# nanoporetech/isONclust2

Measured on AMD Instinct MI355X. Metric: reads/s clustered (sahlin mode, k=11 w=15), higher is better.
Workload: dtype u32

## Files before the change

isonclust2_amd/csrc/ioc_align_gpu.hip:

```cpp
#include <hip/hip_runtime.h>

#include <algorithm>
#include <chrono>
#include <cmath>
#include <cstdint>
#include <cstring>
#include <numeric>
#include <string>
#include <type_traits>
#include <vector>

#include "ioc_align_sink.h"
#include "ioc_internal.h"

namespace {

constexpr int ALN_C = 8;
constexpr int ALN_MAXW = 8;
constexpr int ALN_NEG = INT32_MIN / 4;
constexpr uint32_t ALN_LEN_SHIFT = 26;

struct AlnPairDev {
    uint32_t q_off, n;
    uint32_t r_off, m;
// ... 779 lines not shown
            const int2 x = mylrow[e];
            if (x.x > br || (x.x == br && uint32_t(x.y) < bj)) {
                br = x.x;
                bj = uint32_t(x.y);
            }
        }
        for (int o = 32; o > 0; o >>= 1) {
            const int s = __shfl_xor(br, o);
            const uint32_t j = __shfl_xor(bj, o);
            if (s > br || (s == br && j < bj)) {
                br = s;
                bj = j;
            }
        }
        if (lane == 0) {
            int fin = ALN_NEG;
            uint32_t bi = 0, bjj = m;
            for (uint32_t b2 = 0; b2 < nwaves; ++b2) {
                if (min(n, b2 * tpb * TILE) >= n) break;
                const int2 bb = cross ? X.best[uint64_t(pslot - X.first_pair) * nwaves + b2] : int2{s_best[slot * wpp + b2][0], s_best[slot * wpp + b2][1]};
                if (bb.x > fin) {
                    fin = bb.x;
                    bi = uint32_t(bb.y);
                }
            }
            if (br > fin) {
                fin = br;
                bi = n;
                bjj = bj;
            }
            ends[pid] = int4{fin, int(bi), int(bjj), 0};
        }
    }
}

struct WinStat {
    uint32_t wb = 0, pushed = 0, cnt = 0;
    __device__ __forceinline__ void push(uint32_t bit, uint32_t kmask, uint32_t k, int il)
    {
        wb = ((wb << 1) | bit) & kmask;
        ++pushed;
        if (pushed > k && int(__popc(wb)) >= il) ++cnt;
    }
    __device__ __forceinline__ void push_run(unsigned long long bits, uint32_t m, uint32_t kmask, uint32_t k, int il, uint32_t lane)
    {
        const unsigned long long upto = __brevll(bits << (63u - lane));
        const unsigned long long old = lane + 1u < 64u ? (unsigned long long)wb << (lane + 1u) : 0ull;
        const uint32_t win = uint32_t(old | upto) & kmask;
        const bool hit = lane < m && pushed + lane + 1u > k && int(__popc(win)) >= il;
        cnt += uint32_t(__popcll(__ballot(hit)));
        wb = uint32_t(__builtin_amdgcn_readlane(int(win), int(m - 1u)));
        pushed += m;
    }
    __device__ void blanks(uint32_t g, uint32_t kmask, uint32_t k, int il)
    {
        const uint32_t t = g < k ? g : k;
        for (uint32_t x = 0; x < t; ++x) push(0u, kmask, k, il);
        if (g > t) {
            const uint32_t rest = g - t;
            const uint32_t first_counted = pushed >= k ? 0u : k - pushed;
            pushed += rest;
            if (il <= 0 && rest > first_counted) cnt += rest - first_counted;
        }
    }
};

struct AlnOpsDev {
    uint8_t* buf;
    const uint64_t* end;
    uint32_t* len;
};

struct NoOpsDev {};
template <bool EMIT>
struct OpsOut {
    using Dev = NoOpsDev;
    __device__ __forceinline__ void begin(Dev, uint32_t, uint32_t) {}
    __device__ __forceinline__ void run(unsigned long long, uint32_t, uint32_t) {}
    __device__ __forceinline__ void step(uint8_t, uint32_t) {}
    __device__ __forceinline__ void fill(uint8_t, uint32_t, uint32_t) {}
    __device__ __forceinline__ void end(Dev, uint32_t, uint32_t) {}
    __device__ __forceinline__ void none(Dev, uint32_t) {}
};
template <>
struct OpsOut<true> {
    using Dev = AlnOpsDev;
    uint8_t* cur = nullptr;
    uint8_t* lo = nullptr;
    __device__ __forceinline__ void begin(const Dev& od, uint32_t pid, uint32_t room)
    {
        cur = od.buf + od.end[pid];
        lo = cur - room;
    }
    __device__ __forceinline__ void run(unsigned long long bits, uint32_t m, uint32_t lane)
    {
        if (lane < m && cur - 1 - lane >= lo) cur[-1 - int(lane)] = (bits >> lane) & 1ull ? uint8_t('=') : uint8_t('X');
        cur -= m;
    }
    __device__ __forceinline__ void step(uint8_t op, uint32_t lane)
    {
        if (lane == 0 && cur > lo) cur[-1] = op;
        cur -= 1;
    }
    __device__ __forceinline__ void fill(uint8_t op, uint32_t g, uint32_t lane)
    {
        const uint64_t room = uint64_t(cur > lo ? cur - lo : 0);
        for (uint32_t x = lane; x < g && x < room; x += 64) cur[-1 - int64_t(x)] = op;
// ... 685 lines not shown
    std::vector<uint32_t> rw(size_t(np) * V2_RESUME_WORDS);
    IOC_CHK(c, hipMemcpy(rw.data(), t.resume, rw.size() * 4, hipMemcpyDeviceToHost));
    std::vector<uint32_t> ids(n_pairs);
    for (uint32_t x = 0; x < n_pairs; ++x) ids[x] = order[first_pair + x];
    auto rec = [&](uint32_t pid, uint32_t w) { return rw[size_t(pid) * V2_RESUME_WORDS + w]; };
    auto cost = [&](uint32_t pid) { return (double(rec(pid, 8)) + double(rec(pid, 12))) * 256.0; };
    std::sort(ids.begin(), ids.end(), [&](uint32_t a, uint32_t b) { return cost(a) > cost(b); });
    double sum = 0;
    uint32_t parked = 0;
    for (uint32_t pid : ids) {
        sum += cost(pid);
        parked += rec(pid, 6) ? 1u : 0u;
    }
    fprintf(stderr, "[ioc] k_trace2: %u pairs, %u walks went on in the second launch (deadline %u blocks); mean %.3e cycles (s_memtime), slowest first:\n", n_pairs, parked,
            deadline, sum / n_pairs);
    auto line = [&](const char* tag, uint32_t pid) {
        const AlnPairDev& d = dp[pid];
        fprintf(stderr, "[ioc]   %s pair %u: %.3e + %.3e cycles, n %u m %u, blocks %u (%u on the diagonal) + %u (%u by helpers), tiles %u + %u, gap steps %u, windows %u\n", tag, pid,
                double(rec(pid, 8)) * 256.0, double(rec(pid, 12)) * 256.0, d.n, d.m, rec(pid, 9) & 0xFFFFu, rec(pid, 9) >> 16, rec(pid, 13) & 0xFFFFu, rec(pid, 13) >> 16,
                rec(pid, 10), rec(pid, 14), rec(pid, 11), rec(pid, 15));
    };
    {
        double pk_max = -1e9, un_min = 1e9, pk_sum = 0, un_sum = 0;
        uint32_t npk = 0, nun = 0;
        std::vector<double> pks, uns;
        for (uint32_t pid : ids) {
            const AlnPairDev& d = dp[pid];
            const double q = double(he[pid].x) / double(std::max(1u, std::min(d.n, d.m)));
            if (rec(pid, 6)) {
                pk_max = std::max(pk_max, q), pk_sum += q, ++npk;
                pks.push_back(q);
            } else {
                un_min = std::min(un_min, q), un_sum += q, ++nun;
                uns.push_back(q);
            }
        }
        std::sort(pks.begin(), pks.end());
        std::sort(uns.begin(), uns.end());
        auto qt = [](const std::vector<double>& v, double f) { return v.empty() ? 0.0 : v[std::min(v.size() - 1, size_t(f * double(v.size())))]; };
        fprintf(stderr, "[ioc]   forward score / shorter length: parked walks (%u) mean %.3f, 50 %% %.3f, 90 %% %.3f, 99 %% %.3f, max %.3f | others (%u) min %.3f, 1 %% %.3f, 10 %% %.3f, mean %.3f\n", npk,
                npk ? pk_sum / npk : 0.0, qt(pks, 0.5), qt(pks, 0.9), qt(pks, 0.99), pk_max, nun, un_min, qt(uns, 0.01), qt(uns, 0.1), nun ? un_sum / nun : 0.0);
    }
    for (uint32_t x = 0; x < std::min(n_pairs, 10u); ++x) line("", ids[x]);
    for (uint32_t qx : {n_pairs / 4u, n_pairs / 2u, 3u * n_pairs / 4u}) line("rank", ids[qx]);
    std::vector<uint32_t> sw(size_t(np) * V2_SPLIT_WORDS);
    IOC_CHK(c, hipMemcpy(sw.data(), t.split, sw.size() * 4, hipMemcpyDeviceToHost));
    for (uint32_t l = 0; l < 2u; ++l) {
        auto cyc = [&](uint32_t pid) { return double(rec(pid, l ? 12 : 8)) * 256.0; };
        auto spl = [&](uint32_t pid, uint32_t w) { return sw[size_t(pid) * V2_SPLIT_WORDS + l * (V2_SPLIT_WORDS / 2u) + w]; };
        std::vector<uint32_t> in;
        for (uint32_t pid : ids)
            if (rec(pid, l ? 12 : 8)) in.push_back(pid);
        std::sort(in.begin(), in.end(), [&](uint32_t a, uint32_t b) { return cyc(a) > cyc(b); });
        double tot[8] = {};
        for (uint32_t pid : in) {
            tot[0] += cyc(pid);
            for (uint32_t w = 0; w < 3u; ++w) tot[1 + w] += double(spl(pid, w)) * 256.0;
            tot[4] += double(spl(pid, 3) & 0xFFFFu);
            tot[5] += double(spl(pid, 4));
            tot[6] += double(spl(pid, 5));
            tot[7] += double(spl(pid, 6));
        }
        const double nn = double(std::max<size_t>(1, in.size()));
        fprintf(stderr, "[ioc] split of %s: %zu walks; mean %.3e cycles: blocks %.1f %%, tile recomputation %.1f %%, walk loop %.1f %%; %.1f cycles per tile step; "
                        "blocks of <= 64 columns: %.2f per walk, %.1f %% of the block steps recomputed by walkers\n",
                l ? "k_trace2_help" : "k_trace2", in.size(), tot[0] / nn, 100.0 * tot[1] / std::max(1.0, tot[0]), 100.0 * tot[2] / std::max(1.0, tot[0]),
                100.0 * tot[3] / std::max(1.0, tot[0]), tot[2] / std::max(1.0, tot[7]), tot[4] / nn, 100.0 * tot[6] / std::max(1.0, tot[5]));
        for (size_t x = 0; x < std::min<size_t>(in.size(), 10); ++x) {
            const uint32_t pid = in[x];
            const uint32_t nb = l ? rec(pid, 13) & 0xFFFFu : rec(pid, 9) & 0xFFFFu;
            fprintf(stderr, "[ioc]   split pair %u: %.3e cycles: blocks %.3e, tiles %.3e, walk %.3e; blocks %u (<= 64 columns %u, <= 64 rows %u), own block steps %u (%u in thin), tiles %u, tile steps %u\n",
                    pid, cyc(pid), double(spl(pid, 0)) * 256.0, double(spl(pid, 1)) * 256.0, double(spl(pid, 2)) * 256.0, nb, spl(pid, 3) & 0xFFFFu, spl(pid, 3) >> 16,
                    spl(pid, 4), spl(pid, 5), rec(pid, l ? 14 : 10), spl(pid, 6));
        }
    }
    return IOC_OK;
}

int align_v2_run(ioc_ctx* c, const std::vector<AlnPairDev>& dp, const uint32_t* order, uint32_t cnt, const uint32_t* d_order,
                 const AlnParams& P, int32_t* d_score, uint32_t* d_count, bool corridor, bool* fell_back, OpsRun* ops)
{
    *fell_back = false;
    if (cnt == 0) return IOC_OK;
    int r;
    const auto t_plan0 = std::chrono::steady_clock::now();
    V2Opts o{};
    o.n_cu = compute_units(c);
    uint64_t budget = 0;
    if ((r = ck_budget(c, &budget, ops ? ops->host->pile_bytes() : 0)) != IOC_OK) return r;
    o.guard = P16_GUARD;
    if (const char* e = getenv("IOC_ALIGN_V2_GUARD")) o.guard = std::max(1, std::min(P16_GUARD, atoi(e)));
    o.few_limit = 128;
    if (const char* e = getenv("IOC_ALIGN_V2_FEW")) o.few_limit = uint32_t(std::max(0, atoi(e)));
    if (hipOccupancyMaxActiveBlocksPerMultiprocessor(&o.occ, reinterpret_cast<const void*>(k_fwd2), 64 * V2_WAVES, 0) != hipSuccess) o.occ = 0;
    (void)hipGetLastError();
    if (o.occ < 1) o.occ = 3;

    V2Plan pl;
    pl.cnt = cnt;
    pl.np = uint32_t(dp.size());
    pl.ncouples = (cnt + 1u) / 2u;
    plan_couples(pl, dp, order, corridor_model(c, P, corridor), band_target(pl.ncouples, o.few_limit, o.occ, o.n_cu));
    std::vector<uint64_t> cops;
    if (ops) {
        cops.assign(pl.ncouples, 0);
        for (uint32_t x = 0; x < cnt; ++x) cops[x / 2u] += uint64_t(dp[order[x]].n) + dp[order[x]].m;
    }
    slice_couples(pl, budget, cops);
    std::vector<uint64_t> slice_ops(pl.slices.size(), 0);
    if (ops) {
        ops->end.assign(dp.size(), 0);
        uint64_t most = 0;
        for (size_t si = 0; si < pl.slices.size(); ++si) {
            const uint32_t x0 = 2u * pl.slices[si].first, x1 = std::min(cnt, 2u * (pl.slices[si].first + pl.slices[si].second));
            for (uint32_t x = x0; x < x1; ++x) ops->end[order[x]] = slice_ops[si] += uint64_t(dp[order[x]].n) + dp[order[x]].m;
            most = std::max(most, slice_ops[si]);
        }
        if ((r = ops_reserve(c, *ops, most, dp)) != IOC_OK) return r;
    }
    const auto t_res0 = std::chrono::steady_clock::now();
    IOC_TRY(ioc_reserve(c, c->a_ck, size_t(pl.arena_words) * 4));
    c->tm.align_arena_bytes = int64_t(pl.arena_words) * 4;
    c->tm.align_slices = int32_t(pl.slices.size());
    c->tm.align_version = 2;
    if (getenv("IOC_TRACE"))
        fprintf(stderr, "[ioc]   aligner v2: %u couples, checkpoint arena %.1f MB (%zu slice(s)) reserved in %.3f ms; corridor: %llu of %llu tiles skipped\n", pl.ncouples,
// ... 668 lines not shown
```

isonclust2_amd/csrc/ioc_align_v2.inc:

```

constexpr int CK2 = 512;
constexpr int V2_WAVES = 4;
constexpr int V2_BLK_C = 8;
constexpr int V2_MAX_BANDS = 40;
static_assert(CK2 % TILE == 0 && CK2 == 64 * V2_BLK_C, "block geometry");

struct V2Couple {
    uint32_t pid[2];
    uint32_t nbands, nstrips;
    uint32_t tpb;
    uint32_t flag0;
    uint32_t mpad;
    uint32_t nq;
    uint64_t rdat;
    uint64_t rbase;
    uint64_t cdat;
    uint64_t cbase;
    uint64_t prof;
    uint32_t lrow0[2];
    uint32_t best0[2];
    uint16_t bstart[V2_MAX_BANDS + 1];
    uint16_t plo[V2_MAX_BANDS], phi[V2_MAX_BANDS];
    uint32_t corridor;
    uint16_t probe_band, probe_strip;
// ... 600 lines not shown
        };
        {
            uint32_t s = 0;
            for (; s + 1u < nsteps; s += 2) {
                step(s, std::true_type{});
                step(s + 1u, std::false_type{});
            }
            for (; s < nsteps; ++s) step(s, std::true_type{});
        }
#pragma unroll
        for (int h = 0; h < 2; ++h) {
            if (lastc[h] >= 0) bandbest[par(VP_BEST0 + h) + band] = int2{bc[h], int(bc_i[h])};
            if ((ovf >> h) & 1u) {
                const uint32_t pidh = par(VP_PID0 + h);
                if (pidh != 0xFFFFFFFFu) atomicOr(&ovf_out[pidh], 1u);
            }
        }
        if (lane == 0) {
            unsigned long long cells = 0;
#pragma unroll
            for (int h = 0; h < 2; ++h)
                if (vh[h]) cells += (unsigned long long)(par(VP_RHI0 + h) - r_lo) * (unsigned long long)min(strip_cols, par(VP_M0 + h) - p * strip_cols);
            atomicAdd(cells_done, cells);
        }
        const uint32_t my_flag = uint32_t(__builtin_amdgcn_readfirstlane(int(par(VP_FLAG))));
        asm volatile("s_waitcnt vmcnt(0)" ::: "memory");
        __builtin_amdgcn_fence(__ATOMIC_RELEASE, "agent");
        asm volatile("s_waitcnt vmcnt(0)" ::: "memory");
        __hip_atomic_store(&flags[my_flag], 1u, __ATOMIC_RELAXED, __HIP_MEMORY_SCOPE_AGENT);
        it = v2_dequeue(queue);
    }
}

#define V2_FWD_ARGS                                                                                                                        \
    const AlnPairDev *__restrict__ pairs, const V2Couple *__restrict__ couples, const V2Item *__restrict__ items, uint32_t n_items,        \
        uint32_t *__restrict__ queue, uint32_t *__restrict__ flags, uint32_t *__restrict__ err, const uint8_t *__restrict__ pool, AlnParams P, \
        uint32_t *__restrict__ arena, int2 *__restrict__ lrow, int2 *__restrict__ bandbest, uint32_t *__restrict__ ovf_out, int guard,     \
        const uint4 *__restrict__ prof, unsigned long long *__restrict__ cells_done, uint32_t *__restrict__ prog, uint32_t prog_every
__global__ void __launch_bounds__(64 * V2_WAVES) __attribute__((amdgpu_waves_per_eu(3, 8))) k_fwd2(V2_FWD_ARGS)
{
    v2_fwd_body(pairs, couples, items, n_items, queue, flags, err, pool, P, arena, lrow, bandbest, ovf_out, guard, prof, cells_done, prog, prog_every);
}
__global__ void __launch_bounds__(64 * V2_WAVES) __attribute__((amdgpu_waves_per_eu(2, 2))) k_fwd2_w2(V2_FWD_ARGS)
{
    v2_fwd_body(pairs, couples, items, n_items, queue, flags, err, pool, P, arena, lrow, bandbest, ovf_out, guard, prof, cells_done, prog, prog_every);
}


struct V2PairEnd {
    uint32_t lrow0, best0, nbands, couple;
    int32_t cert;
};
constexpr uint32_t V2_RESUME_WORDS = 16;
constexpr uint32_t V2_SPLIT_WORDS = 16;

__global__ void __launch_bounds__(64)
k_fwd2_probe(const AlnPairDev* __restrict__ pairs, V2Couple* __restrict__ couples, V2PairEnd* __restrict__ pe, const uint32_t* __restrict__ arena, AlnParams P)
{
    V2Couple& cp = couples[blockIdx.x];
    if (!cp.corridor) return;
    const uint32_t lane = threadIdx.x;
    const uint32_t strip_cols = 64u * FW_C;
    const uint32_t R = uint32_t(cp.bstart[cp.probe_band + 1u]) * uint32_t(CK2);
    const uint32_t ckr = R / uint32_t(CK2) - 1u;
    const uint32_t* rh = arena + cp.rdat + uint64_t(2u * ckr) * cp.mpad;
    const int2* rb = reinterpret_cast<const int2*>(arena + cp.rbase) + uint64_t(ckr) * (cp.mpad / 16u);
    bool wrong = false;
    uint32_t nmax = 0, mmax = 0, need = 0, need_raw = 0;
    for (int h = 0; h < 2; ++h) {
        if (cp.pid[h] == 0xFFFFFFFFu) continue;
        const AlnPairDev pr = pairs[cp.pid[h]];
        nmax = max(nmax, pr.n);
        mmax = max(mmax, pr.m);
        const int gd = pr.gap_open - P.gap_extend;
        int mx = INT32_MIN;
        const uint32_t x0 = uint32_t(cp.probe_strip) * strip_cols, x1 = min(pr.m, x0 + strip_cols);
        for (uint32_t x = x0 + lane; x < x1; x += 64) {
            const int2 bb = rb[x / 16u];
            mx = max(mx, v2_half(rh[x], h) + (h ? bb.y : bb.x) + gd - P.gap_extend * int(R + x + 1u));
        }
        for (int o = 32; o > 0; o >>= 1) mx = max(mx, __shfl_xor(mx, o));
        if (pr.n < R || x1 <= x0 || mx < P.match * int(R) / 4) {
            wrong = true;
        } else {
            const float len = float(max(pr.n, pr.m)), rate = float(mx) / float(R);
            const float b = len - 0.97f * rate * float(min(pr.n, pr.m)) / float(P.match) + 512.0f;
            need = max(need, uint32_t(max(b, 0.0f)));
            need_raw = max(need_raw, uint32_t(max(len - rate * float(min(pr.n, pr.m)) / float(P.match), 0.0f)));
        }
    }
    const uint32_t len_max = max(nmax, mmax);
    const uint32_t B0 = cp.b0;
    if (!wrong && need_raw > B0 && need > B0) {
        if (float(need) > 0.4f * float(len_max)) {
            wrong = true;
        } else if (lane == 0) {
            long long beff = 0x7FFFFFFFFFFFll;
            uint32_t skipped = 0;
            for (uint32_t b = 0; b < cp.nbands; ++b) {
                const uint32_t r0 = uint32_t(cp.bstart[b]) * uint32_t(CK2), r1 = min(nmax, uint32_t(cp.bstart[b + 1u]) * uint32_t(CK2));
                const uint32_t c_lo = r0 > need ? r0 - need : 0u;
                const unsigned long long c_hi = min((unsigned long long)mmax, (unsigned long long)r1 + need);
                const uint32_t lo = c_lo / strip_cols, hi = uint32_t((max(c_hi, 1ull) - 1ull) / strip_cols);
                cp.plo[b] = uint16_t(min(lo, uint32_t(cp.plo[b])));
                cp.phi[b] = uint16_t(max(hi, uint32_t(cp.phi[b])));
                skipped += uint32_t(cp.plo[b]) + (cp.nstrips - 1u - uint32_t(cp.phi[b]));
                if (cp.plo[b] > 0) beff = min(beff, (long long)r0 - (long long)cp.plo[b] * strip_cols);
// ... 88 lines not shown
__device__ __forceinline__ int2 v2_ld(const int2* p)
{
    const int x = __hip_atomic_load(&p->x, __ATOMIC_RELAXED, __HIP_MEMORY_SCOPE_AGENT);
    const int y = __hip_atomic_load(&p->y, __ATOMIC_RELAXED, __HIP_MEMORY_SCOPE_AGENT);
    return int2{x, y};
}

constexpr uint32_t V2_NROLE = 5, V2_NHELP = 2 * V2_NROLE, V2_HBUF = 2, V2_HWAVES = 1 + V2_NHELP;
enum V2Help : uint32_t { VH_SEQ = 0, VH_RB, VH_CB, VH_I, VH_J, VH_QUIT, VH_WORK = 8 , VH_SLOT = VH_WORK + 3 * V2_NHELP ,
                         VH_COUNT = VH_SLOT + 3 * V2_NHELP * V2_HBUF };

template <bool HELP, bool EMIT>
__device__ __forceinline__ void trace2_body(const AlnPairDev* __restrict__ pairs, const uint32_t* __restrict__ order, const uint8_t* __restrict__ pool,
                                            const AlnParams& P, const uint32_t* __restrict__ arena, const V2Couple* __restrict__ couples, const V2PairCk* __restrict__ pck,
                                            const int4* __restrict__ ends, V2Scratch* __restrict__ scratch, V2Scratch* __restrict__ hscratch,
                                            uint32_t* __restrict__ resume, uint32_t* __restrict__ park, uint32_t* __restrict__ split,
                                            int32_t* __restrict__ out_score, uint32_t* __restrict__ out_count, const uint32_t count, const uint32_t max_blocks,
                                            const unsigned long long max_cycles, const uint32_t pslot, const uint32_t wv, const uint32_t want,
                                            const typename OpsOut<EMIT>::Dev od)
{
    constexpr int NW = HELP ? int(V2_HWAVES) : TR_WAVES, NDIRS = HELP ? 1 : TR_WAVES;
    constexpr uint32_t B_LEFT = uint32_t(CK2) * 8u, B_Q = uint32_t(CK2) * 4u, B_PROF = 5u * 64u * uint32_t(V2_BLK_C / 4) * 4u;
    constexpr uint32_t D_BYTES = uint32_t(TILE) * uint32_t(TR_C) / 4u * 64u * 2u;
    constexpr uint32_t U_BYTES = (B_LEFT + B_Q + B_PROF) > D_BYTES + uint32_t(TILE) ? (B_LEFT + B_Q + B_PROF) : D_BYTES + uint32_t(TILE);
    __shared__ __attribute__((aligned(16))) uint8_t s_union_all[NW][U_BYTES];
    __shared__ __attribute__((aligned(16))) uint8_t s_tile_all[NDIRS][uint32_t(TILE) * 12u];
    __shared__ uint32_t s_help[VH_COUNT];
    if (pslot >= count) return;
    uint16_t(*dirs)[64] = reinterpret_cast<uint16_t(*)[64]>(&s_union_all[wv][0]);
    int2* const b_left = reinterpret_cast<int2*>(&s_union_all[wv][0]);
    uint32_t* const b_q = reinterpret_cast<uint32_t*>(&s_union_all[wv][B_LEFT]);
    uint32_t* const b_prof = reinterpret_cast<uint32_t*>(&s_union_all[wv][B_LEFT + B_Q]);
    struct TRec {
        int hq, e;
        uint32_t q;
    };
    static_assert(sizeof(TRec) == 12, "a row's record");
    TRec* const s_rec = reinterpret_cast<TRec*>(&s_tile_all[HELP ? 0u : wv][0]);
    uint8_t* const s_rb = &s_union_all[wv][D_BYTES];
    const uint32_t pid = order[pslot];
    const AlnPairDev pr = pairs[pid];
    const V2PairCk ck = pck[pid];
    const int hf = int(ck.half);
    const bool corridor = __builtin_amdgcn_readfirstlane(int(couples[ck.couple].corridor)) != 0;
    uint32_t* const rs = resume + size_t(pid) * V2_RESUME_WORDS;
    {
        const uint32_t fl = uint32_t(__builtin_amdgcn_readfirstlane(int(rs[6])));
        if (HELP ? fl != want : fl == 2u) return;
    }
    V2Scratch* scp = &scratch[pslot];
    const unsigned long long t_begin = __builtin_amdgcn_s_memtime();
    uint32_t n_blocks = 0, n_diag = 0, n_tiles = 0, n_gapsteps = 0;
    unsigned long long t_blk = 0, t_tile = 0, t_walk = 0;
    uint32_t n_thin_c = 0, n_thin_r = 0, n_bsteps = 0, n_bsteps_thin = 0, n_tsteps = 0;
    uint32_t* const sp = split + size_t(pid) * V2_SPLIT_WORDS + (HELP ? V2_SPLIT_WORDS / 2u : 0u);
    auto split_out = [&]() {
        sp[0] = uint32_t(t_blk >> 8);
        sp[1] = uint32_t(t_tile >> 8);
        sp[2] = uint32_t(t_walk >> 8);
        sp[3] = n_thin_c | (n_thin_r << 16);
        sp[4] = n_bsteps;
        sp[5] = n_bsteps_thin;
        sp[6] = n_tsteps;
    };
    const uint32_t n = pr.n, m = pr.m;
    const int go = pr.gap_open, il = pr.ilimit;
    const uint8_t* __restrict__ q = pool + pr.q_off;
    const uint8_t* __restrict__ r = pool + pr.r_off;
    const uint32_t lane = threadIdx.x & 63u;
    const uint32_t k = P.k, kmask = k >= 32 ? 0xFFFFFFFFu : ((1u << k) - 1u);
    const int4 en = ends[pid];
    if (en.w & 3) {
        if (lane == 0) {
            out_score[pid] = (en.w & 1) ? INT32_MIN : INT32_MIN + 1;
            out_count[pid] = 0xFFFFFFFFu;
            OpsOut<EMIT>{}.none(od, pid);
        }
        return;
    }
    const int gd = go - P.gap_extend, ge = P.gap_extend;
    FwdConst K;
    K.ge = ge;
    K.gd = gd;
    K.cm = P.match + 2 * ge + gd;
    K.cx = P.mismatch + 2 * ge + gd;
    uint32_t i = uint32_t(en.y), j = uint32_t(en.z);
    int state = 0;
    WinStat ws;
    OpsOut<EMIT> ops;
    ops.begin(od, pid, n + m);
    if (!EMIT && HELP && want == 1u) {
        i = rs[0];
        j = rs[1];
        state = int(rs[2]);
        ws.wb = rs[3];
        ws.pushed = rs[4];
        ws.cnt = rs[5];
    } else {
        ws.blanks((m - j) + (n - i), kmask, k, il);
        ops.fill('d', m - j, lane);
        ops.fill('i', n - i, lane);
    }
    uint32_t blk_r = 0xFFFFFFFFu, blk_c = 0xFFFFFFFFu;
    auto coarse_row = [&](uint32_t R, uint32_t x) {
        const uint32_t ckr = R / CK2 - 1u;
        const uint32_t* rh = arena + ck.rdat + uint64_t(2u * ckr) * ck.mpad;
        const int2 bb = reinterpret_cast<const int2*>(arena + ck.rbase)[uint64_t(ckr) * (ck.mpad / 16u) + x / 16u];
        const int bs = hf ? bb.y : bb.x;
        return int2{v2_half(rh[x], hf) + bs, v2_half(rh[ck.mpad + x], hf) + bs};
    };
    auto coarse_col = [&](uint32_t C, uint32_t y) {
        const uint64_t e = uint64_t(C / CK2 - 1u) * ck.nq + y / 4u;
        const uint32_t* d = arena + ck.cdat + e * 8u;
        const int2 bb = reinterpret_cast<const int2*>(arena + ck.cbase)[e];
        const int bs = hf ? bb.y : bb.x;
        return int2{v2_half(d[y & 3u], hf) + bs, v2_half(d[4u + (y & 3u)], hf) + bs};
    };

    auto recompute_block_c = [&](auto cpl, const uint32_t Rb, const uint32_t Cb, const uint32_t brows, const uint32_t bcols, V2Scratch& dst) __attribute__((always_inline)) {
        constexpr int BC = decltype(cpl)::value;
        const uint32_t ln = opaque(lane);
        bool top_ok = true, left_ok = true, corner_ok = true;
        if (corridor) {
            const V2Couple& cq = couples[ck.couple];
            auto band_of = [&](uint32_t row) {
                const uint32_t cr = row / uint32_t(CK2);
                uint32_t b = 0;
                while (b + 1u < cq.nbands && uint32_t(cq.bstart[b + 1u]) <= cr) ++b;
                return b;
            };
            auto in = [&](uint32_t b, uint32_t p) { return p >= cq.plo[b] && p <= cq.phi[b]; };
            const uint32_t ps = Cb / (64u * FW_C), pl = Cb ? (Cb - 1u) / (64u * FW_C) : 0u;
            const uint32_t bb = band_of(Rb), bt = Rb ? band_of(Rb - 1u) : 0u;
            if (Rb) top_ok = in(bt, ps);
            if (Cb) left_ok = in(bb, pl);
            if (Rb && Cb) corner_ok = in(bt, pl);
        }
        for (uint32_t x = ln; x <= bcols; x += 64) {
            int2 v;
            if (Rb == 0)
                v = int2{ge * int(Cb + x) - gd, ALN_NEG};
            else if (Cb + x == 0)
                v = int2{ge * int(Rb) - gd, ALN_NEG};
            else if (x ? top_ok : corner_ok)
                v = coarse_row(Rb, Cb + x - 1u);
            else
                v = int2{ALN_NEG, ALN_NEG};
            dst.frow[0][x] = v;
        }
        for (uint32_t y = ln; y < brows; y += 64) {
            int2 v{ge * int(Rb + y + 1) - gd, ALN_NEG};
            if (Cb) v = left_ok ? coarse_col(Cb, Rb + y) : int2{ALN_NEG, ALN_NEG};
            dst.fcol[0][y] = v;
            b_left[y] = v;
            const uint32_t ch = q[Rb + y];
            b_q[y] = (ch == 'A' ? 0u : ch == 'C' ? 1u : ch == 'G' ? 2u : ch == 'T' ? 3u : 4u) * uint32_t(64 * (BC / 4) * 4);
        }
        for (uint32_t y = brows + ln; y < ((brows + 3u) & ~3u) + 4u && y < uint32_t(CK2); y += 64) {
            b_left[y] = int2{0, ALN_NEG};
            b_q[y] = 0;
        }
        const uint32_t jb8 = Cb + ln * BC;
        uint32_t rpk[BC / 4];
#pragma unroll
        for (int c4 = 0; c4 < BC / 4; ++c4) {
            uint32_t w = 0;
#pragma unroll
            for (int e = 0; e < 4; ++e) w |= ref_byte(r, m, pr.rc, jb8 + c4 * 4 + e) << (8 * e);
            rpk[c4] = w;
        }
        {
            const uint32_t bases = 'A' | ('C' << 8) | ('G' << 16) | ('T' << 24);
#pragma unroll
            for (int code = 0; code < 5; ++code) {
                const uint32_t bq = code < 4 ? (bases >> (8 * code)) & 0xFFu : 0x100u;
#pragma unroll
                for (int c4 = 0; c4 < BC / 4; ++c4) {
                    uint32_t w = 0;
#pragma unroll
                    for (int e = 0; e < 4; ++e) w |= uint32_t(((rpk[c4] >> (8 * e)) & 0xFFu) == bq ? K.cm : K.cx) << (8 * e);
                    b_prof[(uint32_t(code) * 64u + ln) * uint32_t(BC / 4) + uint32_t(c4)] = w;
                }
            }
        }
        const uint8_t* bprof = reinterpret_cast<const uint8_t*>(&b_prof[ln * uint32_t(BC / 4)]);
        asm volatile("s_waitcnt vmcnt(0)" ::: "memory");
        tr_wave_sync();
        int Hb[BC], Fb[BC];
        int dgb;
        {
            const uint32_t x0 = ln * BC;
#pragma unroll
            for (int c = 0; c < BC; ++c) {
                int2 v{0, ALN_NEG};
                if (x0 + c + 1 <= bcols) v = v2_ld(&dst.frow[0][x0 + c + 1]);
                Hb[c] = v.x;
                Fb[c] = v.y;
            }
            dgb = x0 <= bcols ? v2_ld(&dst.frow[0][x0]).x : 0;
        }
        const uint32_t nactb = (bcols + BC - 1) / BC;
        const uint32_t nblkb = (brows + FW_R - 1) / FW_R, nstepb = nblkb + nactb - 1u;
        int hl4[FW_R], el4[FW_R];
        uint32_t qc4[FW_R];
#pragma unroll
        for (int rr = 0; rr < FW_R; ++rr) {
            hl4[rr] = 0;
            el4[rr] = ALN_NEG;
            qc4[rr] = 0;
        }
        uint4 nl0 = *reinterpret_cast<const uint4*>(&b_left[0]), nl1 = *reinterpret_cast<const uint4*>(&b_left[2]);
        uint4 nq4 = *reinterpret_cast<const uint4*>(&b_q[0]);
        const bool fine_col_lane = ((ln + 1u) * BC) % TILE == 0 && (ln + 1u) * BC < uint32_t(CK2);
        const uint32_t fine_col_k = ((ln + 1u) * BC) / TILE;
        for (uint32_t s = 0; s < nstepb; ++s) {
            {
                const uint32_t h4[FW_R] = {nl0.x, nl0.z, nl1.x, nl1.z}, e4[FW_R] = {nl0.y, nl0.w, nl1.y, nl1.w},
                               q4[FW_R] = {nq4.x, nq4.y, nq4.z, nq4.w};
#pragma unroll
                for (int rr = 0; rr < FW_R; ++rr) {
                    hl4[rr] = int(from_left_or(uint32_t(hl4[rr]), h4[rr]));
                    el4[rr] = int(from_left_or(uint32_t(el4[rr]), e4[rr]));
                    qc4[rr] = from_left_or(qc4[rr], q4[rr]);
                }
                const uint32_t sn = min(s + 1u, nblkb - 1u) * FW_R;
                nl0 = *reinterpret_cast<const uint4*>(&b_left[sn]);
                nl1 = *reinterpret_cast<const uint4*>(&b_left[sn + 2u]);
                nq4 = *reinterpret_cast<const uint4*>(&b_q[sn]);
            }
            const int bi = int(s) - int(ln);
            if (bi >= 0 && uint32_t(bi) < nblkb && ln < nactb) {
#pragma unroll
                for (int rr = 0; rr < FW_R; ++rr) {
                    const int hl_in = hl4[rr];
                    uint32_t xw[BC / 4];
                    if constexpr (BC == 8) {
                        const uint2 xw2 = *reinterpret_cast<const uint2*>(bprof + qc4[rr]);
                        xw[0] = xw2.x;
                        xw[1] = xw2.y;
                    } else {
                        static_assert(BC == 4, "one or two profile words per ln");
                        xw[0] = *reinterpret_cast<const uint32_t*>(bprof + qc4[rr]);
                    }
                    fwd_cells<BC, true>(Hb, Fb, xw, hl4[rr], el4[rr], dgb, qc4[rr], K);
                    dgb = hl_in;
                }
                const uint32_t y0 = uint32_t(bi) * FW_R;
                if (fine_col_lane) {
#pragma unroll
                    for (int rr = 0; rr < FW_R; ++rr)
                        if (y0 + rr < brows) dst.fcol[fine_col_k][y0 + rr] = int2{hl4[rr], el4[rr]};
                }
                const uint32_t y1 = y0 + FW_R;
                if ((y1 % TILE) == 0 && y1 < uint32_t(CK2) && y1 <= brows) {
                    int2* fr = &dst.frow[y1 / TILE][1u + ln * BC];
#pragma unroll
                    for (int c = 0; c < BC; ++c) fr[c] = int2{Hb[c], Fb[c]};
                    if (ln == 0) dst.frow[y1 / TILE][0] = int2{b_left[y1 - 1u].x, ALN_NEG};
                }
            }
        }
        asm volatile("s_waitcnt vmcnt(0)" ::: "memory");
        tr_wave_sync();
    };

    auto recompute_block = [&](const uint32_t Rb, const uint32_t Cb, const uint32_t brows, const uint32_t bcols, V2Scratch& dst) __attribute__((always_inline)) {
        if (bcols <= 64u * uint32_t(V2_BLK_C / 2))
            recompute_block_c(std::integral_constant<int, V2_BLK_C / 2>{}, Rb, Cb, brows, bcols, dst);
        else
            recompute_block_c(std::integral_constant<int, V2_BLK_C>{}, Rb, Cb, brows, bcols, dst);
    };

    const uint32_t stop_at = EMIT ? 0u : pr.stop_at;
    auto cannot_reach = [&](uint32_t cnt_, uint32_t i_, uint32_t j_) {
        const unsigned long long room = (unsigned long long)(stop_at - cnt_);
        if ((unsigned long long)i_ + j_ + k < room) return true;
        return il >= 1 && (unsigned long long)k * min(i_, j_) + (unsigned long long)((k - 1u) * (k - 1u)) < room * (unsigned long long)il;
    };
    bool decided = stop_at && (ws.cnt >= stop_at || cannot_reach(ws.cnt, i, j));
    const uint32_t help_addr = uint32_t(reinterpret_cast<uintptr_t>(&s_help[0]));
    uint32_t help_seq = 0, n_helped = 0;
    if (HELP) {
        if (wv == 0u) {
            for (uint32_t x = lane; x < uint32_t(VH_COUNT); x += 64) s_help[x] = 0u;
        }
        __syncthreads();
        if (wv != 0u) {
            const uint32_t h = wv - 1u, role = h % V2_NROLE, turn = h / V2_NROLE;
            const int dr = role == 0u ? 1 : role == 2u ? 2 : role == 3u ? 1 : 0;
            const int dc = role == 1u ? 1 : role == 3u ? 1 : role == 4u ? 2 : 0;
            uint32_t last = 0;
            for (;;) {
                uint32_t seq = 0;
                bool quit = false;
                for (uint32_t it = 0; it < (1u << 24); ++it) {
                    quit = v2_par(help_addr + 4u * VH_QUIT) != 0u;
                    seq = v2_par(help_addr + 4u * VH_SEQ);
                    if (quit || seq != last) break;
                    __builtin_amdgcn_s_sleep(8);
                }
                if (quit || seq == last) return;
                const uint32_t qRb = v2_par(help_addr + 4u * VH_RB), qCb = v2_par(help_addr + 4u * VH_CB), qi = v2_par(help_addr + 4u * VH_I),
                               qj = v2_par(help_addr + 4u * VH_J);
                if (v2_par(help_addr + 4u * VH_SEQ) != seq) continue;
                last = seq;
                if ((seq & 1u) != turn) continue;
                if (qRb < uint32_t(dr * CK2) || qCb < uint32_t(dc * CK2)) continue;
                const uint32_t tRb = qRb - uint32_t(dr * CK2), tCb = qCb - uint32_t(dc * CK2);
                const uint32_t trows = dr ? uint32_t(CK2) : min(qi, qRb + uint32_t(CK2)) - qRb;
                const uint32_t tcols = dc ? uint32_t(CK2) : min(qj, qCb + uint32_t(CK2)) - qCb;
                const uint32_t wk = help_addr + 4u * (VH_WORK + 3u * h), buf = (seq >> 1) % V2_HBUF;
                const uint32_t sl = help_addr + 4u * (VH_SLOT + 3u * (h * V2_HBUF + buf));
                v2_lds_store(sl, 0u);
                v2_lds_store(wk + 4u, tRb);
                v2_lds_store(wk + 8u, tCb);
                v2_lds_store(wk, seq);
                recompute_block(tRb, tCb, trows, tcols, hscratch[(size_t(HELP ? blockIdx.x : 0u) * V2_NHELP + size_t(h)) * V2_HBUF + size_t(buf)]);
                asm volatile("s_waitcnt vmcnt(0)" ::: "memory");
                __builtin_amdgcn_fence(__ATOMIC_RELEASE, "agent");
                v2_lds_store(sl + 4u, tRb);
                v2_lds_store(sl + 8u, tCb);
                v2_lds_store(sl, seq);
                v2_lds_store(wk, 0u);
// ... 11 lines not shown
            n_diag += Rb == Cb ? 1u : 0u;
            const uint32_t brows = min(i, Rb + CK2) - Rb, bcols = min(j, Cb + CK2) - Cb;
            if (!HELP && max_blocks && stop_at &&
                (n_blocks > 2u * (stop_at / uint32_t(CK2) + 1u) + max_blocks || (max_cycles && __builtin_amdgcn_s_memtime() - t_begin > max_cycles))) {
                if (lane == 0) {
                    rs[0] = i;
                    rs[1] = j;
                    rs[2] = uint32_t(state);
                    rs[3] = ws.wb;
                    rs[4] = ws.pushed;
                    rs[5] = ws.cnt;
                    rs[6] = 1u;
                    park[1u + atomicAdd(&park[0], 1u)] = pslot;
                    const unsigned long long dt = __builtin_amdgcn_s_memtime() - t_begin;
                    rs[8] = uint32_t(dt >> 8);
                    rs[9] = (n_blocks - 1u) | (n_diag << 16);
                    rs[10] = n_tiles;
                    rs[11] = n_gapsteps;
                    split_out();
                }
                return;
            }
            const unsigned long long t_blk0 = __builtin_amdgcn_s_memtime();
            n_thin_c += bcols <= 64u ? 1u : 0u;
            n_thin_r += brows <= 64u ? 1u : 0u;
            bool have = false;
            if (HELP && help_seq) {
                for (uint32_t it = 0; it < (1u << 22) && !have; ++it) {
                    bool working = false;
                    for (uint32_t h = 0; h < V2_NHELP && !have; ++h) {
                        for (uint32_t bq = 0; bq < V2_HBUF; ++bq) {
                            const uint32_t sl = help_addr + 4u * (VH_SLOT + 3u * (h * V2_HBUF + bq));
                            const uint32_t sq = v2_par(sl);
                            if (sq && sq + 1u >= help_seq && v2_par(sl + 4u) == Rb && v2_par(sl + 8u) == Cb) {
                                scp = &hscratch[(size_t(HELP ? blockIdx.x : 0u) * V2_NHELP + size_t(h)) * V2_HBUF + size_t(bq)];
                                have = true;
                                break;
                            }
                        }
                        const uint32_t wk = help_addr + 4u * (VH_WORK + 3u * h);
                        const uint32_t wq = v2_par(wk);
                        if (!have && wq && wq + 1u >= help_seq && v2_par(wk + 4u) == Rb && v2_par(wk + 8u) == Cb) working = true;
                    }
                    if (have || !working) break;
                    __builtin_amdgcn_s_sleep(4);
                }
                if (have) {
                    __builtin_amdgcn_fence(__ATOMIC_ACQUIRE, "agent");
                    ++n_helped;
                }
            }
            if (!have) {
                scp = &scratch[pslot];
                recompute_block(Rb, Cb, brows, bcols, *scp);
                const uint32_t bcpl = bcols <= 64u * uint32_t(V2_BLK_C / 2) ? uint32_t(V2_BLK_C / 2) : uint32_t(V2_BLK_C);
                const uint32_t bsteps = (brows + FW_R - 1) / FW_R + (bcols + bcpl - 1u) / bcpl - 1u;
                n_bsteps += bsteps;
                n_bsteps_thin += bcols <= 64u ? bsteps : 0u;
            }
            if (HELP) {
                v2_lds_store(help_addr + 4u * VH_RB, Rb);
                v2_lds_store(help_addr + 4u * VH_CB, Cb);
                v2_lds_store(help_addr + 4u * VH_I, i);
                v2_lds_store(help_addr + 4u * VH_J, j);
                ++help_seq;
                v2_lds_store(help_addr + 4u * VH_SEQ, help_seq);
            }
            t_blk += __builtin_amdgcn_s_memtime() - t_blk0;
        }
        int cm = K.cm, cx = K.cx;
        asm volatile("" : "+v"(cm), "+v"(cx));
        const uint32_t kr = (r0 - Rb) / TILE, kc = (c0 - Cb) / TILE;
        ++n_tiles;
        const unsigned long long t_tile0 = __builtin_amdgcn_s_memtime();
        for (uint32_t x = lane; x < rows; x += 64) {
            const int2 v = v2_ld(&scp->fcol[kc][(r0 - Rb) + x]);
            s_rec[x] = TRec{v.x, v.y, q[r0 + x]};
        }
        const uint32_t jb = c0 + lane * TR_C;
        uint32_t rpk[1];
        {
            uint32_t w = 0;
#pragma unroll
            for (int e = 0; e < TR_C; ++e) w |= ref_byte(r, m, pr.rc, jb + e) << (8 * e);
            rpk[0] = w;
        }
        if (TR_C == 4)
            reinterpret_cast<uint32_t*>(s_rb)[lane] = rpk[0];
        else
            reinterpret_cast<uint16_t*>(s_rb)[lane] = uint16_t(rpk[0]);
        uint32_t rb[TR_C];
#pragma unroll
        for (int c = 0; c < TR_C; ++c) rb[c] = (rpk[0] >> (8 * c)) & 0xFFu;
        int Hp[TR_C], F[TR_C];
        int dg;
        {
            const uint32_t x0 = (c0 - Cb) + lane * TR_C;
#pragma unroll
            for (int c = 0; c < TR_C; ++c) {
                int2 v{0, ALN_NEG};
                if (jb + c < m && x0 + c + 1 <= uint32_t(CK2)) v = v2_ld(&scp->frow[kr][x0 + c + 1]);
                Hp[c] = v.x;
                F[c] = v.y;
            }
            dg = x0 <= uint32_t(CK2) ? v2_ld(&scp->frow[kr][x0]).x : 0;
        }
        tr_wave_sync();
        const uint32_t nact = (cols + TR_C - 1) / TR_C;
        const uint32_t nsteps = rows + nact - 1;
        if (lane < nact) {
            int out_h = 0, out_e = ALN_NEG;
// ... 204 lines not shown
```

Before: 62890.

## Recompute thin traceback blocks row-wise and peel block wavefront loop phases

Adds a transposed block recompute path for blocks of at most 64 columns, where lanes own row groups and sweep across columns. Without it, most lanes would idle on such narrow blocks. The column-wise recompute now splits its anti-diagonal loop into ramp-up, steady and ramp-down phases with compile-time activity checks, and makes inactive lanes skip it. It also uses half-height steps for short blocks and writes fine rows and columns with pointer-advanced vector stores. Extra timing counters for own-block cycles are recorded and printed. The new paths add code size and register pressure, and the edge handling could be wrong on corner cases.

New measurement: 64270, median of 6. 1.02x the previous value.

```diff
diff --git a/isonclust2_amd/csrc/ioc_align_gpu.hip b/isonclust2_amd/csrc/ioc_align_gpu.hip
--- a/isonclust2_amd/csrc/ioc_align_gpu.hip
+++ b/isonclust2_amd/csrc/ioc_align_gpu.hip
@@ -855,7 +855,7 @@
         wb = uint32_t(__builtin_amdgcn_readlane(int(win), int(m - 1u)));
         pushed += m;
     }
-    __device__ void blanks(uint32_t g, uint32_t kmask, uint32_t k, int il)
+    __device__ __forceinline__ void blanks(uint32_t g, uint32_t kmask, uint32_t k, int il)
     {
         const uint32_t t = g < k ? g : k;
         for (uint32_t x = 0; x < t; ++x) push(0u, kmask, k, il);
@@ -1647,7 +1647,7 @@
         for (uint32_t pid : ids)
             if (rec(pid, l ? 12 : 8)) in.push_back(pid);
         std::sort(in.begin(), in.end(), [&](uint32_t a, uint32_t b) { return cyc(a) > cyc(b); });
-        double tot[8] = {};
+        double tot[11] = {};
         for (uint32_t pid : in) {
             tot[0] += cyc(pid);
             for (uint32_t w = 0; w < 3u; ++w) tot[1 + w] += double(spl(pid, w)) * 256.0;
@@ -1655,18 +1655,22 @@
             tot[5] += double(spl(pid, 4));
             tot[6] += double(spl(pid, 5));
             tot[7] += double(spl(pid, 6));
+            for (uint32_t w = 0; w < 3u; ++w) tot[8 + w] += double(spl(pid, 7 + w)) * 256.0;
         }
         const double nn = double(std::max<size_t>(1, in.size()));
         fprintf(stderr, "[ioc] split of %s: %zu walks; mean %.3e cycles: blocks %.1f %%, tile recomputation %.1f %%, walk loop %.1f %%; %.1f cycles per tile step; "
                         "blocks of <= 64 columns: %.2f per walk, %.1f %% of the block steps recomputed by walkers\n",
                 l ? "k_trace2_help" : "k_trace2", in.size(), tot[0] / nn, 100.0 * tot[1] / std::max(1.0, tot[0]), 100.0 * tot[2] / std::max(1.0, tot[0]),
                 100.0 * tot[3] / std::max(1.0, tot[0]), tot[2] / std::max(1.0, tot[7]), tot[4] / nn, 100.0 * tot[6] / std::max(1.0, tot[5]));
+        fprintf(stderr, "[ioc]   own blocks: %.1f %% of the blocks' cycles (the rest: waiting for a helper's); %.1f cycles per own block step in blocks of > 64 columns, %.1f in those of <= 64; "
+                        "blocks of <= 64 rows: %.1f %% of the own blocks' cycles\n",
+                100.0 * tot[8] / std::max(1.0, tot[1]), (tot[8] - tot[9]) / std::max(1.0, tot[5] - tot[6]), tot[9] / std::max(1.0, tot[6]), 100.0 * tot[10] / std::max(1.0, tot[8]));
         for (size_t x = 0; x < std::min<size_t>(in.size(), 10); ++x) {
             const uint32_t pid = in[x];
             const uint32_t nb = l ? rec(pid, 13) & 0xFFFFu : rec(pid, 9) & 0xFFFFu;
-            fprintf(stderr, "[ioc]   split pair %u: %.3e cycles: blocks %.3e, tiles %.3e, walk %.3e; blocks %u (<= 64 columns %u, <= 64 rows %u), own block steps %u (%u in thin), tiles %u, tile steps %u\n",
+            fprintf(stderr, "[ioc]   split pair %u: %.3e cycles: blocks %.3e, tiles %.3e, walk %.3e; blocks %u (<= 64 columns %u, <= 64 rows %u), own block steps %u (%u in thin), own block cycles %.3e (%.3e in <= 64 columns, %.3e in <= 64 rows), tiles %u, tile steps %u\n",
                     pid, cyc(pid), double(spl(pid, 0)) * 256.0, double(spl(pid, 1)) * 256.0, double(spl(pid, 2)) * 256.0, nb, spl(pid, 3) & 0xFFFFu, spl(pid, 3) >> 16,
-                    spl(pid, 4), spl(pid, 5), rec(pid, l ? 14 : 10), spl(pid, 6));
+                    spl(pid, 4), spl(pid, 5), double(spl(pid, 7)) * 256.0, double(spl(pid, 8)) * 256.0, double(spl(pid, 9)) * 256.0, rec(pid, l ? 14 : 10), spl(pid, 6));
         }
     }
     return IOC_OK;
diff --git a/isonclust2_amd/csrc/ioc_align_v2.inc b/isonclust2_amd/csrc/ioc_align_v2.inc
--- a/isonclust2_amd/csrc/ioc_align_v2.inc
+++ b/isonclust2_amd/csrc/ioc_align_v2.inc
@@ -676,7 +676,7 @@
     int32_t cert;
 };
 constexpr uint32_t V2_RESUME_WORDS = 16;
-constexpr uint32_t V2_SPLIT_WORDS = 16;
+constexpr uint32_t V2_SPLIT_WORDS = 24;
 
 __global__ void __launch_bounds__(64)
 k_fwd2_probe(const AlnPairDev* __restrict__ pairs, V2Couple* __restrict__ couples, V2PairEnd* __restrict__ pe, const uint32_t* __restrict__ arena, AlnParams P)
@@ -871,6 +871,7 @@
     const unsigned long long t_begin = __builtin_amdgcn_s_memtime();
     uint32_t n_blocks = 0, n_diag = 0, n_tiles = 0, n_gapsteps = 0;
     unsigned long long t_blk = 0, t_tile = 0, t_walk = 0;
+    unsigned long long t_own = 0, t_own_thin_c = 0, t_own_thin_r = 0;
     uint32_t n_thin_c = 0, n_thin_r = 0, n_bsteps = 0, n_bsteps_thin = 0, n_tsteps = 0;
     uint32_t* const sp = split + size_t(pid) * V2_SPLIT_WORDS + (HELP ? V2_SPLIT_WORDS / 2u : 0u);
     auto split_out = [&]() {
@@ -881,6 +882,9 @@
         sp[4] = n_bsteps;
         sp[5] = n_bsteps_thin;
         sp[6] = n_tsteps;
+        sp[7] = uint32_t(t_own >> 8);
+        sp[8] = uint32_t(t_own_thin_c >> 8);
+        sp[9] = uint32_t(t_own_thin_r >> 8);
     };
     const uint32_t n = pr.n, m = pr.m;
     const int go = pr.gap_open, il = pr.ilimit;
@@ -936,10 +940,8 @@
         return int2{v2_half(d[y & 3u], hf) + bs, v2_half(d[4u + (y & 3u)], hf) + bs};
     };
 
-    auto recompute_block_c = [&](auto cpl, const uint32_t Rb, const uint32_t Cb, const uint32_t brows, const uint32_t bcols, V2Scratch& dst) __attribute__((always_inline)) {
-        constexpr int BC = decltype(cpl)::value;
-        const uint32_t ln = opaque(lane);
-        bool top_ok = true, left_ok = true, corner_ok = true;
+    auto block_edges = [&](const uint32_t Rb, const uint32_t Cb, bool& top_ok, bool& left_ok, bool& corner_ok) __attribute__((always_inline)) {
+        top_ok = left_ok = corner_ok = true;
         if (corridor) {
             const V2Couple& cq = couples[ck.couple];
             auto band_of = [&](uint32_t row) {
@@ -955,6 +957,15 @@
             if (Cb) left_ok = in(bb, pl);
             if (Rb && Cb) corner_ok = in(bt, pl);
         }
+    };
+
+    auto recompute_block_c = [&](auto cpl, auto rps, const uint32_t Rb, const uint32_t Cb, const uint32_t brows, const uint32_t bcols, V2Scratch& dst) __attribute__((always_inline)) {
+        constexpr int BC = decltype(cpl)::value;
+        constexpr int RS = decltype(rps)::value;
+        static_assert(RS == FW_R || RS == FW_R / 2, "a step's rows of the left column are one or two 16-byte LDS reads");
+        const uint32_t ln = opaque(lane);
+        bool top_ok, left_ok, corner_ok;
+        block_edges(Rb, Cb, top_ok, left_ok, corner_ok);
         for (uint32_t x = ln; x <= bcols; x += 64) {
             int2 v;
             if (Rb == 0)
@@ -1019,75 +1030,242 @@
             dgb = x0 <= bcols ? v2_ld(&dst.frow[0][x0]).x : 0;
         }
         const uint32_t nactb = (bcols + BC - 1) / BC;
-        const uint32_t nblkb = (brows + FW_R - 1) / FW_R, nstepb = nblkb + nactb - 1u;
-        int hl4[FW_R], el4[FW_R];
-        uint32_t qc4[FW_R];
-#pragma unroll
-        for (int rr = 0; rr < FW_R; ++rr) {
-            hl4[rr] = 0;
-            el4[rr] = ALN_NEG;
-            qc4[rr] = 0;
-        }
-        uint4 nl0 = *reinterpret_cast<const uint4*>(&b_left[0]), nl1 = *reinterpret_cast<const uint4*>(&b_left[2]);
-        uint4 nq4 = *reinterpret_cast<const uint4*>(&b_q[0]);
-        const bool fine_col_lane = ((ln + 1u) * BC) % TILE == 0 && (ln + 1u) * BC < uint32_t(CK2);
-        const uint32_t fine_col_k = ((ln + 1u) * BC) / TILE;
-        for (uint32_t s = 0; s < nstepb; ++s) {
-            {
-                const uint32_t h4[FW_R] = {nl0.x, nl0.z, nl1.x, nl1.z}, e4[FW_R] = {nl0.y, nl0.w, nl1.y, nl1.w},
-                               q4[FW_R] = {nq4.x, nq4.y, nq4.z, nq4.w};
-#pragma unroll
-                for (int rr = 0; rr < FW_R; ++rr) {
-                    hl4[rr] = int(from_left_or(uint32_t(hl4[rr]), h4[rr]));
-                    el4[rr] = int(from_left_or(uint32_t(el4[rr]), e4[rr]));
-                    qc4[rr] = from_left_or(qc4[rr], q4[rr]);
-                }
-                const uint32_t sn = min(s + 1u, nblkb - 1u) * FW_R;
-                nl0 = *reinterpret_cast<const uint4*>(&b_left[sn]);
-                nl1 = *reinterpret_cast<const uint4*>(&b_left[sn + 2u]);
-                nq4 = *reinterpret_cast<const uint4*>(&b_q[sn]);
-            }
-            const int bi = int(s) - int(ln);
-            if (bi >= 0 && uint32_t(bi) < nblkb && ln < nactb) {
-#pragma unroll
-                for (int rr = 0; rr < FW_R; ++rr) {
-                    const int hl_in = hl4[rr];
-                    uint32_t xw[BC / 4];
-                    if constexpr (BC == 8) {
-                        const uint2 xw2 = *reinterpret_cast<const uint2*>(bprof + qc4[rr]);
-                        xw[0] = xw2.x;
-                        xw[1] = xw2.y;
-                    } else {
-                        static_assert(BC == 4, "one or two profile words per ln");
-                        xw[0] = *reinterpret_cast<const uint32_t*>(bprof + qc4[rr]);
-                    }
-                    fwd_cells<BC, true>(Hb, Fb, xw, hl4[rr], el4[rr], dgb, qc4[rr], K);
-                    dgb = hl_in;
-                }
-                const uint32_t y0 = uint32_t(bi) * FW_R;
-                if (fine_col_lane) {
-#pragma unroll
-                    for (int rr = 0; rr < FW_R; ++rr)
-                        if (y0 + rr < brows) dst.fcol[fine_col_k][y0 + rr] = int2{hl4[rr], el4[rr]};
-                }
-                const uint32_t y1 = y0 + FW_R;
-                if ((y1 % TILE) == 0 && y1 < uint32_t(CK2) && y1 <= brows) {
-                    int2* fr = &dst.frow[y1 / TILE][1u + ln * BC];
-#pragma unroll
-                    for (int c = 0; c < BC; ++c) fr[c] = int2{Hb[c], Fb[c]};
-                    if (ln == 0) dst.frow[y1 / TILE][0] = int2{b_left[y1 - 1u].x, ALN_NEG};
-                }
-            }
+        const uint32_t nblkb = (brows + RS - 1) / RS, nstepb = nblkb + nactb - 1u;
+        if (ln >= 1u && ln < uint32_t(CK2 / TILE) && ln * uint32_t(TILE) <= brows) dst.frow[ln][0] = int2{b_left[ln * uint32_t(TILE) - 1u].x, ALN_NEG};
+        if (ln < nactb) {
+            int hl4[RS], el4[RS];
+            uint32_t qc4[RS];
+#pragma unroll
+            for (int rr = 0; rr < RS; ++rr) {
+                hl4[rr] = 0;
+                el4[rr] = ALN_NEG;
+                qc4[rr] = 0;
+            }
+            const int2* lp = b_left;
+            const uint32_t* qp = b_q;
+            uint4 nl0, nl1{}, nq4{};
+            auto next_rows = [&]() __attribute__((always_inline)) {
+                nl0 = *reinterpret_cast<const uint4*>(&lp[0]);
+                if constexpr (RS == 4) {
+                    nl1 = *reinterpret_cast<const uint4*>(&lp[2]);
+                    nq4 = *reinterpret_cast<const uint4*>(&qp[0]);
+                } else {
+                    const uint2 q2 = *reinterpret_cast<const uint2*>(&qp[0]);
+                    nq4.x = q2.x;
+                    nq4.y = q2.y;
+                }
+            };
+            next_rows();
+            const bool fine_col_lane = ((ln + 1u) * BC) % TILE == 0 && (ln + 1u) * BC < uint32_t(CK2);
+            uint8_t* fcp = reinterpret_cast<uint8_t*>(&dst.fcol[fine_col_lane ? ((ln + 1u) * BC) / TILE : 0u][0]) - size_t(ln) * (RS * sizeof(int2));
+            uint8_t* frp = reinterpret_cast<uint8_t*>(&dst.frow[1][1u + ln * BC]);
+            const uint32_t fr_last = min(brows / uint32_t(RS), uint32_t((CK2 - TILE) / RS));
+            uint32_t done = 0u - ln;
+            auto bstep = [&](auto lo, auto hi, auto pre, const uint32_t s) __attribute__((always_inline)) {
+                {
+                    const uint32_t h4[4] = {nl0.x, nl0.z, nl1.x, nl1.z}, e4[4] = {nl0.y, nl0.w, nl1.y, nl1.w},
+                                   q4[4] = {nq4.x, nq4.y, nq4.z, nq4.w};
+#pragma unroll
+                    for (int rr = 0; rr < RS; ++rr) {
+                        hl4[rr] = int(from_left_or(uint32_t(hl4[rr]), h4[rr]));
+                        el4[rr] = int(from_left_or(uint32_t(el4[rr]), e4[rr]));
+                        qc4[rr] = from_left_or(qc4[rr], q4[rr]);
+                    }
+                    if (decltype(pre)::value) {
+                        lp += RS;
+                        qp += RS;
+                        next_rows();
+                    }
+                }
+                ++done;
+                bool act = true;
+                if (decltype(lo)::value) act = ln <= s;
+                if (decltype(hi)::value) act = act && int(ln) > int(s) - int(nblkb);
+                if (act) {
+#pragma unroll
+                    for (int rr = 0; rr < RS; ++rr) {
+                        const int hl_in = hl4[rr];
+                        uint32_t xw[BC / 4];
+                        if constexpr (BC == 8) {
+                            const uint2 xw2 = *reinterpret_cast<const uint2*>(bprof + qc4[rr]);
+                            xw[0] = xw2.x;
+                            xw[1] = xw2.y;
+                        } else {
+                            static_assert(BC == 4, "one or two profile words per ln");
+                            xw[0] = *reinterpret_cast<const uint32_t*>(bprof + qc4[rr]);
+                        }
+                        fwd_cells<BC, true>(Hb, Fb, xw, hl4[rr], el4[rr], dgb, qc4[rr], K);
+                        dgb = hl_in;
+                    }
+                    if (fine_col_lane) {
+                        reinterpret_cast<int4*>(fcp)[0] = int4{hl4[0], el4[0], hl4[1], el4[1]};
+                        if constexpr (RS == 4) reinterpret_cast<int4*>(fcp)[1] = int4{hl4[2], el4[2], hl4[3], el4[3]};
+                    }
+                    if ((done & uint32_t(TILE / RS - 1)) == 0u && done <= fr_last) {
+                        int2* f2 = reinterpret_cast<int2*>(frp);
+                        f2[0] = int2{Hb[0], Fb[0]};
+#pragma unroll
+                        for (int c = 1; c + 1 < BC; c += 2) *reinterpret_cast<int4*>(f2 + c) = int4{Hb[c], Fb[c], Hb[c + 1], Fb[c + 1]};
+                        f2[BC - 1] = int2{Hb[BC - 1], Fb[BC - 1]};
+                        frp += sizeof(dst.frow[0]);
+                    }
+                }
+                fcp += RS * sizeof(int2);
+            };
+            auto run = [&](auto lo, auto hi, auto pre, uint32_t& s, const uint32_t end) __attribute__((always_inline)) {
+                for (; s + 1u < end; s += 2) {
+                    bstep(lo, hi, pre, s);
+                    bstep(lo, hi, pre, s + 1u);
+                }
+                if (s < end) {
+                    bstep(lo, hi, pre, s);
+                    ++s;
+                }
+            };
+            constexpr std::true_type yes{};
+            constexpr std::false_type no{};
+            uint32_t s = 0;
+            run(yes, no, yes, s, min(nactb, nblkb) - 1u);
+            run(no, no, yes, s, nblkb - 1u);
+            run(yes, yes, no, s, nactb - 1u);
+            run(no, yes, no, s, nstepb);
         }
         asm volatile("s_waitcnt vmcnt(0)" ::: "memory");
         tr_wave_sync();
+        return nstepb;
     };
 
+    auto recompute_block_t = [&](const uint32_t Rb, const uint32_t Cb, const uint32_t brows, const uint32_t bcols, V2Scratch& dst) __attribute__((always_inline)) {
+        constexpr int BR = V2_BLK_C;
+        static_assert(BR == 8, "two profile words per lane");
+        const uint32_t ln = opaque(lane);
+        bool top_ok, left_ok, corner_ok;
+        block_edges(Rb, Cb, top_ok, left_ok, corner_ok);
+        int4* const b_top = reinterpret_cast<int4*>(b_q);
+        static_assert((64u + 1u) * sizeof(int4) <= B_Q, "the top row of a block of <= 64 columns");
+        for (uint32_t x = ln; x <= bcols; x += 64) {
+            int2 v;
+            if (Rb == 0)
+                v = int2{ge * int(Cb + x) - gd, ALN_NEG};
+            else if (Cb + x == 0)
+                v = int2{ge * int(Rb) - gd, ALN_NEG};
+            else if (x ? top_ok : corner_ok)
+                v = coarse_row(Rb, Cb + x - 1u);
+            else
+                v = int2{ALN_NEG, ALN_NEG};
+            dst.frow[0][x] = v;
+            uint32_t po = 0;
+            if (x) {
+                const uint32_t ch = ref_byte(r, m, pr.rc, Cb + x - 1u);
+                po = (ch == 'A' ? 0u : ch == 'C' ? 1u : ch == 'G' ? 2u : ch == 'T' ? 3u : 4u) * uint32_t(64 * (BR / 4) * 4);
+            }
+            b_top[x] = int4{v.x, v.y, int(po), 0};
+        }
+        const uint32_t nact = (brows + BR - 1) / BR;
+        for (uint32_t y = ln; y < brows; y += 64) {
+            int2 v{ge * int(Rb + y + 1) - gd, ALN_NEG};
+            if (Cb) v = left_ok ? coarse_col(Cb, Rb + y) : int2{ALN_NEG, ALN_NEG};
+            dst.fcol[0][y] = v;
+            b_left[y] = v;
+        }
+        for (uint32_t y = brows + ln; y < nact * BR; y += 64) b_left[y] = int2{0, ALN_NEG};
+        {
+            uint32_t qpk[BR / 4];
+#pragma unroll
+            for (int c4 = 0; c4 < BR / 4; ++c4) {
+                uint32_t w = 0;
+#pragma unroll
+                for (int e = 0; e < 4; ++e) {
+                    const uint32_t y = ln * BR + c4 * 4 + e;
+                    w |= (y < brows ? uint32_t(q[Rb + y]) : 0u) << (8 * e);
+                }
+                qpk[c4] = w;
+            }
+            const uint32_t bases = 'A' | ('C' << 8) | ('G' << 16) | ('T' << 24);
+#pragma unroll
+            for (int code = 0; code < 5; ++code) {
+                const uint32_t bq = code < 4 ? (bases >> (8 * code)) & 0xFFu : 0x100u;
+#pragma unroll
+                for (int c4 = 0; c4 < BR / 4; ++c4) {
+                    uint32_t w = 0;
+#pragma unroll
+                    for (int e = 0; e < 4; ++e) w |= uint32_t(((qpk[c4] >> (8 * e)) & 0xFFu) == bq ? K.cm : K.cx) << (8 * e);
+                    b_prof[(uint32_t(code) * 64u + ln) * uint32_t(BR / 4) + uint32_t(c4)] = w;
+                }
+            }
+        }
+        const uint8_t* bprof = reinterpret_cast<const uint8_t*>(&b_prof[ln * uint32_t(BR / 4)]);
+        tr_wave_sync();
+        const uint32_t nstep = bcols + nact - 1u;
+        if (ln >= 1u && ln < uint32_t(CK2 / TILE) && ln * uint32_t(TILE) <= brows) dst.frow[ln][0] = int2{b_left[ln * uint32_t(TILE) - 1u].x, ALN_NEG};
+        if (ln < nact) {
+            int Hr[BR], Er[BR];
+#pragma unroll
+            for (int c = 0; c < BR; ++c) {
+                const int2 v = b_left[ln * BR + c];
+                Hr[c] = v.x;
+                Er[c] = v.y;
+            }
+            const int dg_left = b_left[ln ? ln * BR - 1u : 0u].x;
+            int dgt = ln ? dg_left : b_top[0].x;
+            int out_h = 0, out_f = ALN_NEG;
+            uint32_t out_p = 0;
+            const int4* tp = b_top + 1;
+            int4 nrec = tp[0];
+            const bool fine_row_lane = ((ln + 1u) * BR) % TILE == 0 && (ln + 1u) * BR < uint32_t(CK2) && (ln + 1u) * BR <= brows;
+            uint8_t* frp = reinterpret_cast<uint8_t*>(&dst.frow[fine_row_lane ? ((ln + 1u) * BR) / TILE : 0u][1]) - size_t(ln) * sizeof(int2);
+            auto cstep = [&](auto lo, auto hi, auto pre, const uint32_t s) __attribute__((always_inline)) {
+                int hu = int(from_left_or(uint32_t(out_h), uint32_t(nrec.x)));
+                int fu = int(from_left_or(uint32_t(out_f), uint32_t(nrec.y)));
+                const uint32_t po = from_left_or(out_p, uint32_t(nrec.z));
+                if (decltype(pre)::value) nrec = tp[1];
+                ++tp;
+                bool act = true;
+                if (decltype(lo)::value) act = ln <= s;
+                if (decltype(hi)::value) act = act && int(ln) > int(s) - int(bcols);
+                if (act) {
+                    const int hu_in = hu;
+                    const uint2 xw2 = *reinterpret_cast<const uint2*>(bprof + po);
+                    const uint32_t xw[BR / 4] = {xw2.x, xw2.y};
+                    fwd_cells<BR, true>(Hr, Er, xw, hu, fu, dgt, po, K);
+                    dgt = hu_in;
+                    if (fine_row_lane) *reinterpret_cast<int2*>(frp) = int2{hu, fu};
+                }
+                frp += sizeof(int2);
+                out_h = hu;
+                out_f = fu;
+                out_p = po;
+            };
+            auto run = [&](auto lo, auto hi, auto pre, uint32_t& s, const uint32_t end) __attribute__((always_inline)) {
+                for (; s + 1u < end; s += 2) {
+                    cstep(lo, hi, pre, s);
+                    cstep(lo, hi, pre, s + 1u);
+                }
+                if (s < end) {
+                    cstep(lo, hi, pre, s);
+                    ++s;
+                }
+            };
+            constexpr std::true_type yes{};
+            constexpr std::false_type no{};
+            uint32_t s = 0;
+            run(yes, no, yes, s, min(nact, bcols) - 1u);
+            run(no, no, yes, s, bcols - 1u);
+            run(yes, yes, no, s, nact - 1u);
+            run(no, yes, no, s, nstep);
+        }
+        asm volatile("s_waitcnt vmcnt(0)" ::: "memory");
+        tr_wave_sync();
+        return nstep;
+    };
+
     auto recompute_block = [&](const uint32_t Rb, const uint32_t Cb, const uint32_t brows, const uint32_t bcols, V2Scratch& dst) __attribute__((always_inline)) {
+        if (bcols <= 64u) return recompute_block_t(Rb, Cb, brows, bcols, dst);
         if (bcols <= 64u * uint32_t(V2_BLK_C / 2))
-            recompute_block_c(std::integral_constant<int, V2_BLK_C / 2>{}, Rb, Cb, brows, bcols, dst);
-        else
-            recompute_block_c(std::integral_constant<int, V2_BLK_C>{}, Rb, Cb, brows, bcols, dst);
+            return recompute_block_c(std::integral_constant<int, V2_BLK_C / 2>{}, std::integral_constant<int, FW_R>{}, Rb, Cb, brows, bcols, dst);
+        if (brows <= 64u)
+            return recompute_block_c(std::integral_constant<int, V2_BLK_C>{}, std::integral_constant<int, FW_R / 2>{}, Rb, Cb, brows, bcols, dst);
+        return recompute_block_c(std::integral_constant<int, V2_BLK_C>{}, std::integral_constant<int, FW_R>{}, Rb, Cb, brows, bcols, dst);
     };
 
     const uint32_t stop_at = EMIT ? 0u : pr.stop_at;
@@ -1205,11 +1383,14 @@
             }
             if (!have) {
                 scp = &scratch[pslot];
-                recompute_block(Rb, Cb, brows, bcols, *scp);
-                const uint32_t bcpl = bcols <= 64u * uint32_t(V2_BLK_C / 2) ? uint32_t(V2_BLK_C / 2) : uint32_t(V2_BLK_C);
-                const uint32_t bsteps = (brows + FW_R - 1) / FW_R + (bcols + bcpl - 1u) / bcpl - 1u;
+                const unsigned long long t_own0 = __builtin_amdgcn_s_memtime();
+                const uint32_t bsteps = recompute_block(Rb, Cb, brows, bcols, *scp);
+                const unsigned long long t_own1 = __builtin_amdgcn_s_memtime() - t_own0;
                 n_bsteps += bsteps;
                 n_bsteps_thin += bcols <= 64u ? bsteps : 0u;
+                t_own += t_own1;
+                t_own_thin_c += bcols <= 64u ? t_own1 : 0ull;
+                t_own_thin_r += brows <= 64u ? t_own1 : 0ull;
             }
             if (HELP) {
                 v2_lds_store(help_addr + 4u * VH_RB, Rb);
```
